# olegiy/manuscript-ocr

Hardware: NVIDIA B200
Metric: pages/sec (EAST decode+NMS+crop) (higher is better)
Workload: dtype f64 (NMS) / f32 (boxes) / u8 (crops)

## Files before the change

### manuscript-ocr_b200/csrc/crop.cu

```cuda
#include "crop_common.cuh"

namespace {

constexpr int kThreads = 224;
constexpr int kCtasPerSm = 4;
constexpr int kSlots = 3;
constexpr int kSrcBuf = 40 * 1024;
constexpr int kBandsY = 64, kCellsX = 8;

__device__ __forceinline__ void make_plan(const int32_t *cr, int n_pages, int img_h, int img_w, int ih, int iw,
                                          const uint8_t *pages, const uint8_t *const *page_ptrs,
                                          const int32_t *page_hw, Plan &p)
{
    plan_reset(p);
    p.page = cr[0];
    p.x1 = cr[1];
    p.y1 = cr[2];
    p.w = cr[3] - cr[1];
    p.h = cr[4] - cr[2];
    p.ok = p.page >= 0 && p.page < n_pages;
    if (!p.ok) return;
    const int H = page_ptrs ? page_hw[2 * p.page] : img_h, W = page_ptrs ? page_hw[2 * p.page + 1] : img_w;
    const uint8_t *page0 = page_ptrs ? page_ptrs[p.page] : pages + (size_t)p.page * img_h * (size_t)img_w * 3;
    p.ok = page0 != nullptr && H > 0 && W > 0 && p.w > 0 && p.h > 0 && p.x1 >= 0 && p.y1 >= 0 && cr[3] <= W && cr[4] <= H;
    if (!p.ok) return;
    const int w = p.w, h = p.h;
    plan_resize(w, h, ih, iw, p);
    const size_t stride = (size_t)W * 3;
    p.stride = (int)stride;
    p.src = page0 + (size_t)p.y1 * stride + (size_t)p.x1 * 3;
    const uintptr_t first = reinterpret_cast<uintptr_t>(p.src);
    const uintptr_t last_end = first + (size_t)(h - 1) * stride + (size_t)w * 3;
    const uintptr_t lo = reinterpret_cast<uintptr_t>(page_ptrs ? page0 : pages);
    const uintptr_t hi = page_ptrs ? lo + (size_t)H * stride : lo + (size_t)n_pages * img_h * (size_t)img_w * 3;
    const int mis = (stride & 15) == 0 ? (int)(first & 15) : 15;
    const int pitch = (mis + w * 3 + 15) & ~15;
    const bool fits = (size_t)pitch * h + 16 <= (size_t)kSrcBuf;
    const bool tail_ok = ((last_end + 15) & ~(uintptr_t)15) <= hi;
    if (fits && tail_ok && (lo & 15) == 0) {
        p.staged = 1;
        p.pitch = pitch;
    }
    p.fast = p.staged && p.w < 65536 && p.h < 65536 &&
             ((p.interp == 3 && p.scale_x < 2.999 && p.scale_y < 2.999) || (p.interp == 2 && p.isx == 2 && p.isy == 2));
}

__device__ __forceinline__ int crop_bucket(const Plan &p, const int32_t *page_hw, int img_h, int img_w, int n_pages)
{
    const int H = page_hw ? page_hw[2 * p.page] : img_h, W = page_hw ? page_hw[2 * p.page + 1] : img_w;
    const int by = min(kBandsY - 1, (int)(((int64_t)p.y1 * kBandsY) / max(H, 1)));
    const int bx = min(kCellsX - 1, (int)(((int64_t)p.x1 * kCellsX) / max(W, 1)));
    return (min(p.page, n_pages - 1) * kBandsY + by) * kCellsX + bx;
}

__global__ void __launch_bounds__(256) crop_plan_kernel(const uint8_t *__restrict__ pages,
                                                        const uint8_t *const *__restrict__ page_ptrs,
                                                        const int32_t *__restrict__ page_hw, int n_pages, int img_h,
                                                        int img_w, const int32_t *__restrict__ crops,
                                                        const int32_t *__restrict__ n_crops_dev,
                                                        const int32_t *__restrict__ range, int64_t crops_cap, int ih,
                                                        int iw, Plan *__restrict__ plans, int32_t *__restrict__ hist)
{
    ms_pdl_wait();
    int64_t begin = range ? range[0] : 0;
    int64_t n_crops = range ? range[1] : *n_crops_dev;
    if (n_crops > crops_cap) n_crops = crops_cap;
    for (int64_t i = begin + (int64_t)blockIdx.x * blockDim.x + threadIdx.x; i < n_crops;
         i += (int64_t)gridDim.x * blockDim.x) {
        Plan p;
        make_plan(crops + i * 5, n_pages, img_h, img_w, ih, iw, pages, page_ptrs, page_hw, p);
        plans[i] = p;
        if (p.fast) atomicAdd(&hist[crop_bucket(p, page_ptrs ? page_hw : nullptr, img_h, img_w, n_pages)], 1);
    }
}

__global__ void __launch_bounds__(1024) crop_bucket_scan_kernel(int32_t *__restrict__ hist, int n_buckets,
                                                                int32_t *__restrict__ n_work)
{
    ms_pdl_wait();
    __shared__ int s_warp[32];
    __shared__ int s_carry;
    const int lane = threadIdx.x & 31, warp = threadIdx.x >> 5;
    if (threadIdx.x == 0) s_carry = 0;
    __syncthreads();
    for (int tile = 0; tile < n_buckets; tile += 32 * 1024) {
        const int lo = tile + (int)threadIdx.x * 32;
        int v[32];
        if (lo + 32 <= n_buckets) {
            const int4 *q = reinterpret_cast<const int4 *>(hist + lo);
#pragma unroll
            for (int i = 0; i < 8; i++) {
                const int4 x = q[i];
                v[4 * i] = x.x, v[4 * i + 1] = x.y, v[4 * i + 2] = x.z, v[4 * i + 3] = x.w;
            }
        } else {
#pragma unroll
            for (int i = 0; i < 32; i++) v[i] = lo + i < n_buckets ? hist[lo + i] : 0;
        }
        int sum = 0;
#pragma unroll
        for (int i = 0; i < 32; i++) {
            const int c = v[i];
            v[i] = sum;
            sum += c;
        }
        int incl = sum;
#pragma unroll
        for (int o = 1; o < 32; o <<= 1) {
            const int u = __shfl_up_sync(0xffffffffu, incl, o);
            if (lane >= o) incl += u;
        }
        if (lane == 31) s_warp[warp] = incl;
        __syncthreads();
        const int carry = s_carry;
        if (warp == 0) {
            const int w = s_warp[lane];
            int wi = w;
#pragma unroll
            for (int o = 1; o < 32; o <<= 1) {
                const int u = __shfl_up_sync(0xffffffffu, wi, o);
                if (lane >= o) wi += u;
            }
            s_warp[lane] = wi - w;
            if (lane == 31) s_carry = carry + wi;
        }
        __syncthreads();
        const int base = carry + s_warp[warp] + incl - sum;
        if (lo + 32 <= n_buckets) {
            int4 *q = reinterpret_cast<int4 *>(hist + lo);
#pragma unroll
            for (int i = 0; i < 8; i++) q[i] = make_int4(base + v[4 * i], base + v[4 * i + 1], base + v[4 * i + 2], base + v[4 * i + 3]);
        } else {
#pragma unroll
            for (int i = 0; i < 32; i++)
                if (lo + i < n_buckets) hist[lo + i] = base + v[i];
        }
        __syncthreads();
    }
    if (threadIdx.x == 0) *n_work = s_carry;
}

__global__ void __launch_bounds__(256) crop_bucket_scatter_kernel(const Plan *__restrict__ plans,
                                                                  const int32_t *__restrict__ page_hw, int n_pages,
                                                                  int img_h, int img_w,
                                                                  const int32_t *__restrict__ n_crops_dev,
                                                                  const int32_t *__restrict__ range, int64_t crops_cap,
                                                                  int32_t *__restrict__ cursors, StageDesc *__restrict__ work)
{
    ms_pdl_wait();
    int64_t begin = range ? range[0] : 0;
    int64_t n_crops = range ? range[1] : *n_crops_dev;
    if (n_crops > crops_cap) n_crops = crops_cap;
    for (int64_t i = begin + (int64_t)blockIdx.x * blockDim.x + threadIdx.x; i < n_crops;
         i += (int64_t)gridDim.x * blockDim.x) {
        const Plan p = plans[i];
        if (p.fast) {
            StageDesc d;
            d.src = p.src;
            d.stride = p.stride;
            d.pitch = p.pitch;
            d.row_bytes = 3 * p.w;
            d.rows = p.h;
            d.ci = (int)i;
            work[atomicAdd(&cursors[crop_bucket(p, page_hw, img_h, img_w, n_pages)], 1)] = d;
        }
    }
}

constexpr int kProducerWarps = 2;
constexpr int kConsumerWarps = kThreads / 32 - kProducerWarps;

template <class T, bool kWriteU8>
__global__ void __launch_bounds__(kThreads, kCtasPerSm)
    crop_resize_pad_kernel(const Plan *__restrict__ plans, const StageDesc *__restrict__ work,
                           const int32_t *__restrict__ n_work_dev, int32_t *__restrict__ ticket, int ring_bytes, int ih,
                           int iw, T *__restrict__ batch, uint8_t *__restrict__ canvas_out, int vec_ok,
                           uint8_t *__restrict__ redo)
{
    ms_pdl_wait();
    extern __shared__ __align__(128) unsigned char smem[];
    const int tab_n = area_tab_words(ih, iw);
    uint32_t *tabs = reinterpret_cast<uint32_t *>(smem + ring_bytes);
    __shared__ StageSlots<kSlots> s_stage;
    __shared__ int s_meta[kSlots][8];

    const int warp = threadIdx.x >> 5, lane = threadIdx.x & 31;
    const int plane = ih * iw;
    stage_init(s_stage, kConsumerWarps);

    if (warp == 0) {
        stage_copy_warp(s_stage, smem, ring_bytes, work, *n_work_dev, ticket);
        return;
    }
    if (warp == 1) {
        for (int k = 0;; k++) {
            const int s = k % kSlots;
            const int ci = stage_wait_tick(s_stage, k);
            if (ci < 0) break;
            const Plan p = plans[ci];
            const bool two = p.interp == 2;
            const bool x3 = two || __all_sync(0xffffffffu, build_tables(p, tabs + (size_t)s * tab_n, tab_n, iw, lane));
            if (lane == 0) {
                s_meta[s][0] = p.nw;
                s_meta[s][1] = p.nh;
                s_meta[s][2] = p.y0;
                s_meta[s][3] = p.pitch;
                s_meta[s][4] = (int)(reinterpret_cast<uintptr_t>(p.src) & 15);
                s_meta[s][5] = p.stride & 15;
                s_meta[s][6] = two ? 2 : (x3 ? 1 : 0);
                s_meta[s][7] = strip_height<kConsumerWarps * 32>(p.nw, p.nh);
            }
            __syncwarp();
            if (lane == 0) mbar_arrive(&s_stage.full[s]);
            write_padding<T, kWriteU8>(p.nw, p.nh, p.y0, ih, iw, kHasBatch<T> ? batch + (size_t)ci * 3 * plane : nullptr,
                                               kWriteU8 ? canvas_out + (size_t)ci * 3 * plane : nullptr, vec_ok, lane, 32);
        }
        return;
    }

    const int ct = (warp - kProducerWarps) * 32 + lane;
    constexpr int kCT = kConsumerWarps * 32;
    for (int k = 0;; k++) {
        const int s = k % kSlots;
        const int64_t ci = stage_wait_full(s_stage, k);
        if (ci < 0) break;
        const int nw = s_meta[s][0], nh = s_meta[s][1], y0 = s_meta[s][2];
        const uint32_t pitch = (uint32_t)s_meta[s][3], a0 = (uint32_t)s_meta[s][4], sstep = (uint32_t)s_meta[s][5];
        const int G = s_meta[s][7];
        const uint32_t stage_off = (uint32_t)s_stage.off[s];
        T *dstf = kHasBatch<T> ? batch + (size_t)ci * 3 * plane : nullptr;
        uint8_t *dstu = kWriteU8 ? canvas_out + (size_t)ci * 3 * plane : nullptr;
        const uint32_t *tab = tabs + (size_t)s * tab_n;
        bool bad = false;
        if (s_meta[s][6] == 2)
            area2x2_pixels<T, kWriteU8, kCT>(smem, stage_off, pitch, a0, sstep, ih, iw, nw, nh, y0, dstf, dstu, ct);
        else if (sstep == 0)
            bad = s_meta[s][6] == 1 ? area4_strips<T, kWriteU8, kCT, 3, true>(smem, stage_off, pitch, a0, 0u, tab, tab_n, ih,
                                                                                 iw, nw, nh, y0, dstf, dstu, ct, G)
                               : area4_strips<T, kWriteU8, kCT, 4, true>(smem, stage_off, pitch, a0, 0u, tab, tab_n, ih,
                                                                                 iw, nw, nh, y0, dstf, dstu, ct, G);
        else
            bad = s_meta[s][6] == 1 ? area4_strips<T, kWriteU8, kCT, 3>(smem, stage_off, pitch, a0, sstep, tab, tab_n, ih, iw,
                                                                           nw, nh, y0, dstf, dstu, ct, G)
                               : area4_strips<T, kWriteU8, kCT, 4>(smem, stage_off, pitch, a0, sstep, tab, tab_n, ih, iw,
                                                                           nw, nh, y0, dstf, dstu, ct, G);
        if (bad) redo[ci] = 1;
        stage_release(s_stage, s);
    }
}

__global__ void __launch_bounds__(256) crop_generic_list_kernel(const Plan *__restrict__ plans,
                                                                const int32_t *__restrict__ n_crops_dev,
                                                                const int32_t *__restrict__ range, int64_t crops_cap,
                                                                const uint8_t *__restrict__ redo,
                                                                int32_t *__restrict__ list, int32_t *__restrict__ list_n)
{
    ms_pdl_wait();
    const int64_t begin = range ? range[0] : 0;
    int64_t n_crops = range ? range[1] : *n_crops_dev;
    if (n_crops > crops_cap) n_crops = crops_cap;
    for (int64_t ci = begin + (int64_t)blockIdx.x * blockDim.x + threadIdx.x; ci < n_crops;
         ci += (int64_t)gridDim.x * blockDim.x)
        if (!plans[ci].fast || redo[ci]) list[atomicAdd(list_n, 1)] = (int32_t)ci;
}

constexpr int kGenericMaxTab = 1024;

template <class T, bool kWriteU8>
__global__ void __launch_bounds__(256) crop_generic_kernel(const Plan *__restrict__ plans,
                                                           const int32_t *__restrict__ list,
                                                           const int32_t *__restrict__ list_n, int ih, int iw,
                                                           T *__restrict__ batch,
                                                           uint8_t *__restrict__ canvas_out, int vec_ok)
{
    ms_pdl_wait();
    __shared__ AxisEnt s_tab[kGenericMaxTab];
    const int plane = ih * iw;
    const int todo = *list_n;
    for (int li = blockIdx.x; li < todo; li += gridDim.x) {
        const int64_t ci = list[li];
        Plan p = plans[ci];
        if (!p.ok) p.nw = p.nh = 0;
        T *dstf = kHasBatch<T> ? batch + (size_t)ci * 3 * plane : nullptr;
        uint8_t *dstu = kWriteU8 ? canvas_out + (size_t)ci * 3 * plane : nullptr;
        write_padding<T, kWriteU8>(p, ih, iw, dstf, dstu, vec_ok, threadIdx.x, blockDim.x);
        const bool need_tab = p.ok && (p.interp == 1 || p.interp == 3);
        const bool tab_ok = need_tab && p.nw + p.nh <= kGenericMaxTab;
        __syncthreads();
        if (tab_ok) fill_axis_table(p, s_tab);
        __syncthreads();
        resample_canvas<T, kWriteU8>(p, PitchedSrc{p.src, (size_t)p.stride}, s_tab, tab_ok, need_tab, ih, iw, dstf,
                                             dstu);
    }
}

__global__ void __launch_bounds__(256) detector_input_kernel(const uint8_t *__restrict__ page, int H, int W, int th,
                                                             int tw, float *__restrict__ out_f32,
                                                             uint8_t *__restrict__ out_u8)
{
    ms_pdl_wait();
    const double scale_x = 1.0 / ((double)tw / (double)W), scale_y = 1.0 / ((double)th / (double)H);
    const bool same = (th == H && tw == W);
    const size_t plane = (size_t)th * tw;
    const PitchedSrc src{page, (size_t)W * 3};
    Plan p;
    p.interp = same ? 0 : 1;
    p.isx = p.isy = 0;
    for (size_t i = (size_t)blockIdx.x * blockDim.x + threadIdx.x; i < plane; i += (size_t)gridDim.x * blockDim.x) {
        const int dy = (int)(i / tw), dx = (int)(i - (size_t)dy * tw);
        AxisEnt ex = {}, ey = {};
        if (!same) {
            ex = linear_entry_x(dx, scale_x, W);
            ey = linear_entry_y(dy, scale_y, H);
        }
        unsigned char o0, o1, o2;
        resample_px(p, dx, dy, src, ex, ey, o0, o1, o2);
        if (out_f32) {
            out_f32[i] = ((float)o0 / 255.0f - 0.5f) / 0.5f;
            out_f32[plane + i] = ((float)o1 / 255.0f - 0.5f) / 0.5f;
            out_f32[2 * plane + i] = ((float)o2 / 255.0f - 0.5f) / 0.5f;
        }
        if (out_u8) {
            out_u8[i * 3] = o0;
            out_u8[i * 3 + 1] = o1;
            out_u8[i * 3 + 2] = o2;
        }
    }
}

}

int msk_detector_input(ms_ctx *ctx, const uint8_t *page, int img_h, int img_w, int target_h, int target_w,
                       float *out_f32, uint8_t *out_u8, cudaStream_t st)
{
    if (!page || img_h <= 0 || img_w <= 0 || target_h <= 0 || target_w <= 0 || (!out_f32 && !out_u8)) {
        ms_set_error("detector_input: bad arguments");
        return MS_ERR_INVALID;
    }
    const size_t n = (size_t)target_h * target_w;
    size_t grid = (n + 255) / 256;
    if (grid > (size_t)ctx->num_sms * 16) grid = (size_t)ctx->num_sms * 16;
    ms_launch(detector_input_kernel, (int)grid, 256, 0, st, page, img_h, img_w, target_h, target_w, out_f32, out_u8);
    MS_LAUNCH_CHECK(ctx);
    return MS_OK;
}

static size_t crop_bucket_count(int n_pages)
{
    size_t b = (size_t)(n_pages > 0 ? n_pages : 1) * kBandsY * kCellsX;
    return b > ((size_t)1 << 22) ? ((size_t)1 << 22) : b;
}

size_t msk_crop_scratch(int64_t crops_cap, int n_pages)
{
    const size_t n = (size_t)(crops_cap > 0 ? crops_cap : 0);
    return n * sizeof(Plan) + n + n * sizeof(int32_t) + n * sizeof(StageDesc) + crop_bucket_count(n_pages) * sizeof(int32_t) + 8192;
}

int msk_crop(ms_ctx *ctx, const uint8_t *pages, int n_pages, int img_h, int img_w, const int32_t *crops,
             const int32_t *n_crops, const int32_t *range, int64_t crops_cap, int out_h, int out_w, void *batch,
             int batch_dtype, uint8_t *canvas_u8, ms_bump bump, cudaStream_t st, const uint8_t *const *page_ptrs, const int32_t *page_hw)
{
    if (crops_cap <= 0 || n_pages <= 0) return MS_OK;
    const bool ragged = page_ptrs != nullptr && page_hw != nullptr;
    if (out_h <= 0 || out_w <= 0 || (!ragged && (img_h <= 0 || img_w <= 0 || !pages)) || (!batch && !canvas_u8)) {
        ms_set_error("crop: bad arguments");
        return MS_ERR_INVALID;
    }
    if ((int64_t)out_h * out_w > (1 << 20)) {
        ms_set_error("crop: canvas %dx%d too large", out_h, out_w);
        return MS_ERR_INVALID;
    }
    const size_t tab_bytes = (size_t)kSlots * (size_t)area_tab_words(out_h, out_w) * sizeof(uint32_t);
    const size_t min_ring = (size_t)kSrcBuf + 128;
    int per_sm = kCtasPerSm;
    while (per_sm > 1 && (227 * 1024) / per_sm < (int)(tab_bytes + min_ring + 1024 + 512)) per_sm--;
    if ((227 * 1024) / per_sm < (int)(tab_bytes + min_ring + 1024 + 512)) {
        ms_set_error("crop: canvas %dx%d needs %zu bytes of shared memory", out_h, out_w, tab_bytes + min_ring);
        return MS_ERR_INVALID;
    }
    size_t ring = ((size_t)(227 * 1024) / per_sm - 1024 - 512 - tab_bytes) & ~(size_t)127;
    if (ring > 96 * 1024) ring = 96 * 1024;
    const size_t smem = ring + tab_bytes;
    const int n_buckets = (int)crop_bucket_count(n_pages);
    Plan *plans = bump.take<Plan>((size_t)crops_cap);
    uint8_t *redo = bump.take<uint8_t>((size_t)crops_cap);
    int32_t *glist = bump.take<int32_t>((size_t)crops_cap);
    StageDesc *work = bump.take<StageDesc>((size_t)crops_cap);
    int32_t *hist = bump.take<int32_t>((size_t)n_buckets);
    int32_t *cnt = bump.take<int32_t>(4);
    if (!plans || !redo || !cnt) {
        ms_set_error("crop: scratch too small");
        return MS_ERR_CAPACITY;
    }
    int32_t *glist_n = cnt, *n_work = cnt + 1, *ticket = cnt + 2;
    MS_CUDA(cudaMemsetAsync(redo, 0, (size_t)crops_cap, st));
    MS_CUDA(cudaMemsetAsync(hist, 0, (size_t)n_buckets * sizeof(int32_t), st));
    MS_CUDA(cudaMemsetAsync(cnt, 0, 4 * sizeof(int32_t), st));
    int64_t lgrid = (crops_cap + 255) / 256;
    if (lgrid > (int64_t)ctx->num_sms * 8) lgrid = (int64_t)ctx->num_sms * 8;
    ms_launch(crop_plan_kernel, (int)lgrid, 256, 0, st, pages, ragged ? page_ptrs : nullptr, page_hw, n_pages, img_h, img_w, crops,
                                                 n_crops, range, crops_cap, out_h, out_w, plans, hist);
    MS_LAUNCH_CHECK(ctx);
    ms_launch(crop_bucket_scan_kernel, 1, 1024, 0, st, hist, n_buckets, n_work);
    MS_LAUNCH_CHECK(ctx);
    ms_launch(crop_bucket_scatter_kernel, (int)lgrid, 256, 0, st, plans, ragged ? page_hw : nullptr, n_pages, img_h, img_w, n_crops,
                                                           range, crops_cap, hist, work);
    MS_LAUNCH_CHECK(ctx);
    int64_t grid = (int64_t)ctx->num_sms * per_sm;
    if (grid > crops_cap) grid = crops_cap;
    int64_t ggrid = (int64_t)ctx->num_sms * 8;
    if (ggrid > crops_cap) ggrid = crops_cap;
    return launch_for_outputs(batch, batch_dtype, canvas_u8, [&](auto bt, auto u8) {
        using T = typename decltype(bt)::type;
        constexpr bool kU8 = decltype(u8)::value;
        T *out = static_cast<T *>(batch);
        const int vec_ok = batch_vec_ok<T>(batch, out_w);
        MS_TRY(ms_allow_smem(ctx, batch_slot<T, kU8>(MS_SMEM_CROP_U8), crop_resize_pad_kernel<T, kU8>, (int)smem));
        ms_launch(crop_resize_pad_kernel<T, kU8>, (int)grid, kThreads, smem, st, plans, work, n_work, ticket, (int)ring,
                  out_h, out_w, out, canvas_u8, vec_ok, redo);
        MS_LAUNCH_CHECK(ctx);
        ms_launch(crop_generic_list_kernel, (int)lgrid, 256, 0, st, plans, n_crops, range, crops_cap, redo, glist, glist_n);
        MS_LAUNCH_CHECK(ctx);
        ms_launch(crop_generic_kernel<T, kU8>, (int)ggrid, 256, 0, st, plans, glist, glist_n, out_h, out_w, out,
                  canvas_u8, vec_ok);
        MS_LAUNCH_CHECK(ctx);
        return MS_OK;
    });
}
```

### manuscript-ocr_b200/csrc/crop_common.cuh

```cuda
#pragma once
#include <cuda_bf16.h>
#include <cuda_fp16.h>

#include <type_traits>

#include "ms_internal.cuh"

namespace {

struct NoBatch {};
template <class T>
constexpr bool kHasBatch = !std::is_same<T, NoBatch>::value;

template <class T>
__device__ __forceinline__ T to_batch(float v);
template <>
__device__ __forceinline__ float to_batch<float>(float v) { return v; }
template <>
__device__ __forceinline__ __half to_batch<__half>(float v) { return __float2half_rn(v); }
template <>
__device__ __forceinline__ __nv_bfloat16 to_batch<__nv_bfloat16>(float v) { return __float2bfloat16_rn(v); }
__device__ __forceinline__ uint32_t batch_bits(__half v) { return __half_as_ushort(v); }
__device__ __forceinline__ uint32_t batch_bits(__nv_bfloat16 v) { return __bfloat16_as_ushort(v); }

template <class T>
__device__ __forceinline__ void store_norm(T *p, float v)
{
    __stcs(p, to_batch<T>((v - 127.5f) * (1.0f / 127.5f)));
}

__device__ __forceinline__ uint32_t smem_u32(const void *p) { return (uint32_t)__cvta_generic_to_shared(p); }

__device__ __forceinline__ void mbar_init(uint64_t *bar, int count)
{
    asm volatile("mbarrier.init.shared::cta.b64 [%0], %1;" ::"r"(smem_u32(bar)), "r"(count));
}
__device__ __forceinline__ void mbar_expect_tx(uint64_t *bar, uint32_t bytes)
{
    asm volatile("mbarrier.arrive.expect_tx.shared::cta.b64 _, [%0], %1;" ::"r"(smem_u32(bar)), "r"(bytes) : "memory");
}
__device__ __forceinline__ void mbar_wait(uint64_t *bar, uint32_t parity)
{
    asm volatile(
        "{\n"
        ".reg .pred p;\n"
        "mbarrier.try_wait.parity.shared::cta.b64 p, [%0], %1;\n"
        "@p bra DONE_%=;\n"
        "WAIT_%=:\n"
        "nanosleep.u32 %2;\n"
        "mbarrier.try_wait.parity.shared::cta.b64 p, [%0], %1;\n"
        "@!p bra WAIT_%=;\n"
        "DONE_%=:\n"
        "}\n" ::"r"(smem_u32(bar)),
        "r"(parity), "r"(100u)
        : "memory");
}
__device__ __forceinline__ void tma_bulk_g2s(void *dst_smem, const void *src_gmem, uint32_t bytes, uint64_t *bar)
{
    asm volatile("cp.async.bulk.shared::cluster.global.mbarrier::complete_tx::bytes [%0], [%1], %2, [%3];" ::"r"(
                     smem_u32(dst_smem)),
                 "l"(src_gmem), "r"(bytes), "r"(smem_u32(bar))
                 : "memory");
}
__device__ __forceinline__ void mbar_arrive(uint64_t *bar)
{
    asm volatile("mbarrier.arrive.shared::cta.b64 _, [%0];" ::"r"(smem_u32(bar)) : "memory");
}


struct __align__(16) StageDesc {
    const uint8_t *src;
    int stride;
    int pitch;
    int row_bytes;
    int rows;
    int ci;
};
static_assert(sizeof(StageDesc) == 32, "the copy warp loads a descriptor as two uint4");

template <int kSlots>
struct StageSlots {
    uint64_t full[kSlots], empty[kSlots], tick[kSlots];
    int ci[kSlots];
    int off[kSlots];
    int pitch[kSlots];
};

template <int kSlots>
__device__ __forceinline__ uint32_t stage_parity(int k)
{
    return (uint32_t)((k / kSlots) & 1);
}

template <int kSlots>
__device__ __forceinline__ void stage_init(StageSlots<kSlots> &ss, int consumer_warps)
{
    if (threadIdx.x == 0) {
#pragma unroll
        for (int i = 0; i < kSlots; i++) {
            mbar_init(&ss.full[i], 2);
            mbar_init(&ss.empty[i], consumer_warps);
            mbar_init(&ss.tick[i], 1);
        }
        asm volatile("fence.mbarrier_init.release.cluster;" ::: "memory");
    }
    __syncthreads();
}

template <int kSlots>
__device__ __forceinline__ void stage_copy_warp(StageSlots<kSlots> &ss, unsigned char *ring, int ring_bytes,
                                                const StageDesc *__restrict__ work, int n_work, int32_t *ticket)
{
    const int lane = threadIdx.x & 31;
    int q_off[kSlots], q_len[kSlots];
#pragma unroll
    for (int i = 0; i < kSlots; i++) q_off[i] = q_len[i] = 0;
    int head = 0;
    int oldest = 0;
    auto release_oldest = [&]() {
        mbar_wait(&ss.empty[oldest % kSlots], stage_parity<kSlots>(oldest));
        q_len[oldest % kSlots] = 0;
        oldest++;
    };
    auto load_desc = [&](int t) {
        StageDesc d;
        if (t < n_work) {
            const uint4 *q = reinterpret_cast<const uint4 *>(work + t);
            const uint4 a = q[0], b = q[1];
            d.src = reinterpret_cast<const uint8_t *>(((uint64_t)a.y << 32) | a.x);
            d.stride = (int)a.z;
            d.pitch = (int)a.w;
            d.row_bytes = (int)b.x;
            d.rows = (int)b.y;
            d.ci = (int)b.z;
        } else {
            d.src = nullptr;
            d.stride = d.pitch = d.row_bytes = d.rows = 0;
            d.ci = -1;
        }
        return d;
    };
    int t1 = 0;
    if (lane == 0) t1 = atomicAdd(ticket, 1);
    StageDesc cur = load_desc(__shfl_sync(0xffffffffu, t1, 0));
    if (lane == 0) t1 = atomicAdd(ticket, 1);
    for (int k = 0;; k++) {
        const int s = k % kSlots;
        const StageDesc nxt = load_desc(__shfl_sync(0xffffffffu, t1, 0));
        if (lane == 0 && cur.ci >= 0) t1 = atomicAdd(ticket, 1);
        while (oldest + kSlots <= k) release_oldest();
        if (cur.ci < 0) {
            if (lane == 0) {
                ss.ci[s] = -1;
                mbar_arrive(&ss.tick[s]);
                mbar_arrive(&ss.full[s]);
            }
            return;
        }
        const int need = (cur.pitch * cur.rows + 16 + 127) & ~127;
        int off;
        for (;;) {
            auto free_at = [&](int c) {
                bool ok = c + need <= ring_bytes;
#pragma unroll
                for (int i = 0; i < kSlots; i++) ok = ok && (q_len[i] == 0 || c + need <= q_off[i] || q_off[i] + q_len[i] <= c);
                return ok;
            };
            if (free_at(head)) {
                off = head;
                break;
            }
            if (free_at(0)) {
                off = 0;
                break;
            }
            release_oldest();
        }
        q_off[s] = off;
        q_len[s] = need;
        head = off + need;
        if (lane == 0) {
            ss.ci[s] = cur.ci;
            ss.off[s] = off;
            ss.pitch[s] = cur.pitch;
            mbar_arrive(&ss.tick[s]);
        }
        uint32_t bytes = 0;
        {
            const size_t stride = (size_t)cur.stride;
            unsigned char *buf = ring + off;
            for (int r = lane; r < cur.rows; r += 32) {
                const uint8_t *g = cur.src + (size_t)r * stride;
                const uint32_t a = (uint32_t)(reinterpret_cast<uintptr_t>(g) & 15);
                const uint32_t sz = (a + (uint32_t)cur.row_bytes + 15) & ~15u;
                tma_bulk_g2s(buf + (size_t)r * cur.pitch, g - a, sz, &ss.full[s]);
                bytes += sz;
            }
#pragma unroll
            for (int o = 16; o > 0; o >>= 1) bytes += __shfl_xor_sync(0xffffffffu, bytes, o);
        }
        if (lane == 0) mbar_expect_tx(&ss.full[s], bytes);
        cur = nxt;
    }
}

template <int kSlots>
__device__ __forceinline__ int stage_wait_tick(StageSlots<kSlots> &ss, int k)
{
    const int s = k % kSlots;
    mbar_wait(&ss.tick[s], stage_parity<kSlots>(k));
    const int ci = ss.ci[s];
    if (ci < 0 && (threadIdx.x & 31) == 0) mbar_arrive(&ss.full[s]);
    return ci;
}

template <int kSlots>
__device__ __forceinline__ int stage_wait_full(StageSlots<kSlots> &ss, int k)
{
    mbar_wait(&ss.full[k % kSlots], stage_parity<kSlots>(k));
    return ss.ci[k % kSlots];
}

template <int kSlots>
__device__ __forceinline__ void stage_release(StageSlots<kSlots> &ss, int s)
{
    __syncwarp();
    if ((threadIdx.x & 31) == 0) mbar_arrive(&ss.empty[s]);
}

struct Plan {
    int page, x1, y1, w, h;
    int nw, nh, y0;
    int interp;
    int isx, isy;
    int ok;
    int staged;
    int fast;
    int pitch;
    int stride;
    const uint8_t *src;
    double scale_x, scale_y;
};

__device__ __forceinline__ void plan_reset(Plan &p)
{
    p.page = p.x1 = p.y1 = p.w = p.h = 0;
    p.nw = p.nh = p.y0 = p.interp = p.isx = p.isy = 0;
    p.ok = p.staged = p.fast = p.pitch = p.stride = 0;
    p.src = nullptr;
    p.scale_x = p.scale_y = 1.0;
}

struct AxisEnt {
    int s0;
    int n;
    int nfirst;
    int nmid;
    float af, am, al;
    int pad;
};

__device__ __forceinline__ int cv_round(float v) { return __float2int_rn(v); }
__device__ __forceinline__ unsigned char sat_u8(int v) { return (unsigned char)min(max(v, 0), 255); }

__device__ __forceinline__ void plan_resize(int w, int h, int ih, int iw, Plan &p)
{
    double s1 = (double)ih / (double)max(h, 1), s2 = (double)iw / (double)max(w, 1);
// ... 337 lines not shown
    asm("mul.rn.f32x2 %0, %1, %2;" : "=l"(r) : "l"(a), "l"(b));
    return r;
}
__device__ __forceinline__ unsigned long long bytes2_f32(uint32_t va, uint32_t sa, uint32_t vb, uint32_t sb)
{
    const unsigned long long magic = f2_pack(-8388608.0f, -8388608.0f);
    return f2_add(f2_pack_bits(__byte_perm(va, 0x4B000000u, sa), __byte_perm(vb, 0x4B000000u, sb)), magic);
}

template <int kTaps>
__device__ __forceinline__ void hrow_area4(const unsigned char *smem_base, uint32_t o, const float4 wx, float &b0,
                                           float &b1, float &b2)
{
    const uint32_t *smem32 = reinterpret_cast<const uint32_t *>(smem_base);
    const uint32_t wi = o >> 2, sh = (o & 3u) * 8u;
    const uint32_t q0 = smem32[wi], q1 = smem32[wi + 1], q2 = smem32[wi + 2];
    const uint32_t q3 = kTaps > 3 ? smem32[wi + 3] : 0u;
    const uint32_t u0 = __funnelshift_r(q0, q1, sh), u1 = __funnelshift_r(q1, q2, sh), u2 = __funnelshift_r(q2, q3, sh);
    float p00, p01, p02, p10, p11, p12, p20, p21, p22;
    f2_unpack(f2_mul(bytes2_f32(u0, 0x7650, u0, 0x7651), f2_pack(wx.x, wx.x)), p00, p01);
    f2_unpack(f2_mul(bytes2_f32(u0, 0x7652, u0, 0x7653), f2_pack(wx.x, wx.y)), p02, p10);
    f2_unpack(f2_mul(bytes2_f32(u1, 0x7650, u1, 0x7651), f2_pack(wx.y, wx.y)), p11, p12);
    f2_unpack(f2_mul(bytes2_f32(u1, 0x7652, u1, 0x7653), f2_pack(wx.z, wx.z)), p20, p21);
    if (kTaps > 3) {
        float p30, p31, p32;
        f2_unpack(f2_mul(bytes2_f32(u2, 0x7650, u2, 0x7651), f2_pack(wx.z, wx.w)), p22, p30);
        f2_unpack(f2_mul(bytes2_f32(u2, 0x7652, u2, 0x7653), f2_pack(wx.w, wx.w)), p31, p32);
        b0 = ((p00 + p10) + p20) + p30;
        b1 = ((p01 + p11) + p21) + p31;
        b2 = ((p02 + p12) + p22) + p32;
    } else {
        p22 = byte_f32(u2, 0x7650) * wx.z;
        b0 = (p00 + p10) + p20;
        b1 = (p01 + p11) + p21;
        b2 = (p02 + p12) + p22;
    }
}

__host__ __device__ inline int area_tab_ybase(int iw) { return (5 * iw + 3) & ~3; }
__host__ __device__ inline int area_tab_words(int ih, int iw) { return area_tab_ybase(iw) + 8 * ih; }

__device__ __forceinline__ bool build_tables(const Plan &p, uint32_t *tab, int tab_n, int iw, int tid,
                                             int nthreads = 32)
{
    float *tw = reinterpret_cast<float *>(tab);
    bool x3 = true;
    const double inv_x = 1.0 / p.scale_x, inv_y = 1.0 / p.scale_y;
    for (int t = tid; t < p.nw + p.nh; t += nthreads) {
        const bool isx = t < p.nw;
        const int d = isx ? t : t - p.nw;
        const AxisEnt e = isx ? area_entry(d, p.scale_x, p.w, inv_x) : area_entry(d, p.scale_y, p.h, inv_y);
        const bool fits = e.n <= 4 && e.s0 >= 0 && e.s0 < 65536;
        x3 = x3 && !(isx && e.n > 3);
        const uint32_t packed = fits ? ((uint32_t)e.s0 | ((uint32_t)e.n << 16)) : 0xffff0000u;
        if (isx) {
            tab[d] = packed;
#pragma unroll
            for (int k = 0; k < 4; k++) tw[(size_t)(1 + k) * iw + d] = k < e.n ? area_weight(e, k) : 0.f;
        } else {
            uint32_t *rec = tab + area_tab_ybase(iw) + 8 * d;
            rec[0] = packed;
#pragma unroll
            for (int k = 0; k < 4; k++) reinterpret_cast<float *>(rec)[4 + k] = k < e.n ? area_weight(e, k) : 0.f;
        }
    }
    return x3;
}

template <int kCT>
__device__ __forceinline__ int strip_height(int nw, int nh)
{
    int G = 1, best = 0x7fffffff;
    for (int g = 8; g >= 1; g >>= 1) {
        const int items = ((nh + g - 1) / g) * nw;
        const int cost = ((items + kCT - 1) / kCT) * (2 * g + 1);
        if (cost < best) {
            best = cost;
            G = g;
        }
    }
    return G;
}

template <class T, bool kWriteU8, int kCT>
__device__ __forceinline__ void area2x2_pixels(const unsigned char *smem, uint32_t stage_off, uint32_t pitch, uint32_t a0,
                                               uint32_t sstep, int ih, int iw, int nw, int nh, int y0, T *dstf,
                                               uint8_t *dstu, int ct)
{
    const int plane = ih * iw;
    const uint32_t magic = 0xFFFFFFFFu / (uint32_t)nw + 1u;
    for (int t = ct; t < nw * nh; t += kCT) {
        const int dy = nw == 1 ? t : (int)__umulhi((uint32_t)t, magic), dx = t - dy * nw;
        int s0 = 0, s1 = 0, s2 = 0;
#pragma unroll
        for (int yy = 0; yy < 2; yy++) {
            const uint32_t r = (uint32_t)(2 * dy + yy);
            const unsigned char *row = smem + stage_off + r * pitch + ((a0 + r * sstep) & 15u) + 6u * (uint32_t)dx;
            s0 += row[0] + row[3];
            s1 += row[1] + row[4];
            s2 += row[2] + row[5];
        }
        const int o0 = (s0 + 2) >> 2, o1 = (s1 + 2) >> 2, o2 = (s2 + 2) >> 2;
        const int at = (y0 + dy) * iw + dx;
        if constexpr (kHasBatch<T>) {
            store_norm(dstf + at, (float)o0);
            store_norm(dstf + plane + at, (float)o1);
            store_norm(dstf + 2 * plane + at, (float)o2);
        }
        if (kWriteU8) {
            dstu[(size_t)at * 3] = (unsigned char)o0;
            dstu[(size_t)at * 3 + 1] = (unsigned char)o1;
            dstu[(size_t)at * 3 + 2] = (unsigned char)o2;
        }
    }
}

template <class T, bool kWriteU8, int kCT, int kTaps, bool kAligned = false>
__device__ __forceinline__ bool area4_strips(const unsigned char *smem, uint32_t stage_off, uint32_t pitch, uint32_t a0,
                                             uint32_t sstep, const uint32_t *tab, int tab_n, int ih, int iw, int nw,
                                             int nh, int y0, T *dstf, uint8_t *dstu, int ct, int G_in = 0,
                                             int dy_lo = 0, int dy_hi = -1)
{
    const int plane = ih * iw;
    const int G = G_in > 0 ? G_in : strip_height<kCT>(nw, nh);
    if (dy_hi < 0) dy_hi = nh;
    const int nitems = ((dy_hi - dy_lo + G - 1) / G) * nw;
    const uint32_t magic = 0xFFFFFFFFu / (uint32_t)nw + 1u;
    const float *tw = reinterpret_cast<const float *>(tab);
    bool bad = false;
    for (int t = ct; t < nitems; t += kCT) {
        const int grp = nw == 1 ? t : (int)__umulhi((uint32_t)t, magic), dx = t - grp * nw;
        const uint32_t px = tab[dx];
        bad = bad || (px >> 16) > 4u;
        const float4 wx = make_float4(tw[iw + dx], tw[2 * iw + dx], tw[3 * iw + dx], tw[4 * iw + dx]);
        const uint32_t xoff = stage_off + (px & 0xffffu) * 3u;
        int last_r = -1;
        float b0 = 0.f, b1 = 0.f, b2 = 0.f;
        const int dy_first = dy_lo + grp * G, dy_end = min(dy_hi, dy_first + G);
        T *orow = kHasBatch<T> ? dstf + (size_t)(y0 + dy_first) * iw + dx : nullptr;
        for (int dy = dy_first; dy < dy_end; dy++) {
            const uint32_t *yrec = tab + area_tab_ybase(iw) + 8 * dy;
            const uint32_t py = yrec[0];
            bad = bad || (py >> 16) > 4u;
            const int ys0 = (int)(py & 0xffffu), yn = min((int)(py >> 16), 4);
            const float4 wy4 = *reinterpret_cast<const float4 *>(yrec + 4);
            const float wyv[4] = {wy4.x, wy4.y, wy4.z, wy4.w};
            const uint32_t rbase = xoff + (uint32_t)ys0 * pitch;
            if (ys0 != last_r) {
                const uint32_t mis = (kAligned || sstep == 0) ? a0 : ((a0 + (uint32_t)ys0 * sstep) & 15u);
                hrow_area4<kTaps>(smem, rbase + mis, wx, b0, b1, b2);
            }
            float sum0 = wyv[0] * b0, sum1 = wyv[0] * b1, sum2 = wyv[0] * b2;
#pragma unroll
            for (int j = 1; j < 4; j++) {
                if (j < yn) {
                    const uint32_t r = (uint32_t)(ys0 + j);
                    const uint32_t mis = (kAligned || sstep == 0) ? a0 : ((a0 + r * sstep) & 15u);
                    hrow_area4<kTaps>(smem, rbase + (uint32_t)j * pitch + mis, wx, b0, b1, b2);
                    sum0 += wyv[j] * b0;
                    sum1 += wyv[j] * b1;
                    sum2 += wyv[j] * b2;
                }
            }
            last_r = ys0 + yn - 1;
            const float f0 = rintf(sum0), f1 = rintf(sum1), f2 = rintf(sum2);
            const int at = (y0 + dy) * iw + dx;
            if constexpr (kHasBatch<T>) {
                store_norm(orow, f0);
                store_norm(orow + plane, f1);
                store_norm(orow + 2 * plane, f2);
                orow += iw;
            }
            if (kWriteU8) {
                dstu[(size_t)at * 3] = sat_u8((int)f0);
                dstu[(size_t)at * 3 + 1] = sat_u8((int)f1);
                dstu[(size_t)at * 3 + 2] = sat_u8((int)f2);
            }
        }
    }
    return bad;
}

template <class T>
struct BatchType {
    using type = T;
};

template <class Launch>
int launch_for_outputs(const void *batch, int batch_dtype, const uint8_t *canvas_u8, Launch &&launch)
{
    if (!batch) return launch(BatchType<NoBatch>{}, std::true_type{});
    switch (batch_dtype) {
    case MS_DTYPE_F32:
        return canvas_u8 ? launch(BatchType<float>{}, std::true_type{}) : launch(BatchType<float>{}, std::false_type{});
    case MS_DTYPE_F16:
        return canvas_u8 ? launch(BatchType<__half>{}, std::true_type{}) : launch(BatchType<__half>{}, std::false_type{});
    case MS_DTYPE_BF16:
        return canvas_u8 ? launch(BatchType<__nv_bfloat16>{}, std::true_type{})
                         : launch(BatchType<__nv_bfloat16>{}, std::false_type{});
    }
    ms_set_error("crop: unknown batch dtype %d", batch_dtype);
    return MS_ERR_INVALID;
}

template <class T, bool kWriteU8>
constexpr ms_smem_slot batch_slot(ms_smem_slot first)
{
    const int t = std::is_same<T, float>::value ? 0 : std::is_same<T, __half>::value ? 1 : 2;
    return (ms_smem_slot)(first + (kHasBatch<T> ? 1 + 2 * t + (kWriteU8 ? 1 : 0) : 0));
}

template <class T>
int batch_vec_ok(const void *batch, int out_w)
{
    return (out_w % kBatchVec<T> == 0 && (reinterpret_cast<uintptr_t>(batch) & 15) == 0) ? 1 : 0;
}

}
```

Measured before the change: 28280.

## Stage resized crops in shared-memory tiles and add a dedicated canvas writer warp

Consumer warps now write resized pixels as bytes into a per-slot shared-memory tile instead of scattering normalized values straight to global memory. A new writer warp then streams the whole padded canvas (normalization, padding and u8 copy) with vectorized streaming stores, replacing the separate padding pass. The copy warp's ring allocator now reserves room for both the source and the tile, with extra barriers for tile completion and drain, and the block grows from 224 to 256 threads. This aims at coalesced global writes and at overlapping output writeback with compute. The cost is more shared memory per crop, so fewer crops take the fast staged path, plus added synchronization and a possible bottleneck on the single writer warp.

```diff
diff --git a/manuscript-ocr_b200/csrc/crop.cu b/manuscript-ocr_b200/csrc/crop.cu
--- a/manuscript-ocr_b200/csrc/crop.cu
+++ b/manuscript-ocr_b200/csrc/crop.cu
@@ -2,7 +2,7 @@
 
 namespace {
 
-constexpr int kThreads = 224;
+constexpr int kThreads = 256;
 constexpr int kCtasPerSm = 4;
 constexpr int kSlots = 3;
 constexpr int kSrcBuf = 40 * 1024;
@@ -10,7 +10,7 @@
 
 __device__ __forceinline__ void make_plan(const int32_t *cr, int n_pages, int img_h, int img_w, int ih, int iw,
                                           const uint8_t *pages, const uint8_t *const *page_ptrs,
-                                          const int32_t *page_hw, Plan &p)
+                                          const int32_t *page_hw, int ring_bytes, Plan &p)
 {
     plan_reset(p);
     p.page = cr[0];
@@ -35,7 +35,8 @@
     const uintptr_t hi = page_ptrs ? lo + (size_t)H * stride : lo + (size_t)n_pages * img_h * (size_t)img_w * 3;
     const int mis = (stride & 15) == 0 ? (int)(first & 15) : 15;
     const int pitch = (mis + w * 3 + 15) & ~15;
-    const bool fits = (size_t)pitch * h + 16 <= (size_t)kSrcBuf;
+    const bool fits = (size_t)pitch * h + 16 <= (size_t)ring_bytes &&
+                      stage_src_need(pitch, h) + stage_tile_need(tile_bytes(p.nw, p.nh)) <= ring_bytes;
     const bool tail_ok = ((last_end + 15) & ~(uintptr_t)15) <= hi;
     if (fits && tail_ok && (lo & 15) == 0) {
         p.staged = 1;
@@ -59,7 +60,8 @@
                                                         int img_w, const int32_t *__restrict__ crops,
                                                         const int32_t *__restrict__ n_crops_dev,
                                                         const int32_t *__restrict__ range, int64_t crops_cap, int ih,
-                                                        int iw, Plan *__restrict__ plans, int32_t *__restrict__ hist)
+                                                        int iw, int ring_bytes, Plan *__restrict__ plans,
+                                                        int32_t *__restrict__ hist)
 {
     ms_pdl_wait();
     int64_t begin = range ? range[0] : 0;
@@ -68,7 +70,7 @@
     for (int64_t i = begin + (int64_t)blockIdx.x * blockDim.x + threadIdx.x; i < n_crops;
          i += (int64_t)gridDim.x * blockDim.x) {
         Plan p;
-        make_plan(crops + i * 5, n_pages, img_h, img_w, ih, iw, pages, page_ptrs, page_hw, p);
+        make_plan(crops + i * 5, n_pages, img_h, img_w, ih, iw, pages, page_ptrs, page_hw, ring_bytes, p);
         plans[i] = p;
         if (p.fast) atomicAdd(&hist[crop_bucket(p, page_ptrs ? page_hw : nullptr, img_h, img_w, n_pages)], 1);
     }
@@ -162,12 +164,131 @@
             d.row_bytes = 3 * p.w;
             d.rows = p.h;
             d.ci = (int)i;
+            d.tile_bytes = tile_bytes(p.nw, p.nh);
             work[atomicAdd(&cursors[crop_bucket(p, page_hw, img_h, img_w, n_pages)], 1)] = d;
         }
     }
 }
 
-constexpr int kProducerWarps = 2;
+__device__ __forceinline__ void norm2(uint32_t va, uint32_t sa, uint32_t vb, uint32_t sb, float &lo, float &hi)
+{
+    const unsigned long long half = f2_pack(-127.5f, -127.5f), inv = f2_pack(1.0f / 127.5f, 1.0f / 127.5f);
+    f2_unpack(f2_mul(f2_add(bytes2_f32(va, sa, vb, sb), half), inv), lo, hi);
+}
+template <class T>
+__device__ __forceinline__ uint32_t pack2(float lo, float hi);
+template <>
+__device__ __forceinline__ uint32_t pack2<__half>(float lo, float hi)
+{
+    const __half2 h = __floats2half2_rn(lo, hi);
+    return *reinterpret_cast<const uint32_t *>(&h);
+}
+template <>
+__device__ __forceinline__ uint32_t pack2<__nv_bfloat16>(float lo, float hi)
+{
+    const __nv_bfloat162 h = __floats2bfloat162_rn(lo, hi);
+    return *reinterpret_cast<const uint32_t *>(&h);
+}
+template <int kW>
+__device__ __forceinline__ void pad_bytes(uint32_t (&w)[kW], int keep)
+{
+#pragma unroll
+    for (int j = 0; j < kW; j++) {
+        const int kb = keep - 4 * j;
+        if (kb < 4) w[j] |= kb <= 0 ? 0xFFFFFFFFu : 0xFFFFFFFFu << (8 * kb);
+    }
+}
+
+template <class T, bool kWriteU8>
+__device__ __forceinline__ void write_canvas(const unsigned char *tile, int nw, int nh, int y0, int ih, int iw, T *dstf,
+                                             uint8_t *dstu, int vec_ok, int lane)
+{
+    const uint32_t tp = (uint32_t)tile_pitch(nw);
+    if constexpr (kHasBatch<T>) {
+        if (vec_ok) {
+            constexpr int kV = kBatchVec<T>, kW = 3 * kV / 4;
+            const int V = iw / kV, n = ih * V;
+            uint4 *out = reinterpret_cast<uint4 *>(dstf);
+            int y = 0, v = lane;
+            while (v >= V) v -= V, y++;
+            for (int i = lane; i < n; i += 32) {
+                const int x = v * kV;
+                uint32_t w[kW];
+#pragma unroll
+                for (int j = 0; j < kW; j++) w[j] = 0xFFFFFFFFu;
+                if ((unsigned)(y - y0) < (unsigned)nh && x < nw) {
+                    const unsigned char *px = tile + (uint32_t)(y - y0) * tp + 3u * (uint32_t)x;
+                    if constexpr (kW == 6) {
+#pragma unroll
+                        for (int j = 0; j < 3; j++) {
+                            const uint2 q = reinterpret_cast<const uint2 *>(px)[j];
+                            w[2 * j] = q.x, w[2 * j + 1] = q.y;
+                        }
+                    } else {
+#pragma unroll
+                        for (int j = 0; j < kW; j++) w[j] = reinterpret_cast<const uint32_t *>(px)[j];
+                    }
+                    pad_bytes(w, 3 * (nw - x));
+                }
+#pragma unroll
+                for (int c = 0; c < 3; c++) {
+                    uint32_t o[4];
+#pragma unroll
+                    for (int e = 0; e < kV; e += 2) {
+                        constexpr int kSel = 0x7650;
+                        const int ka = 3 * e + c, kb = ka + 3;
+                        float lo, hi;
+                        norm2(w[ka >> 2], kSel | (ka & 3), w[kb >> 2], kSel | (kb & 3), lo, hi);
+                        if constexpr (sizeof(T) == 4) {
+                            o[e] = __float_as_uint(lo);
+                            o[e + 1] = __float_as_uint(hi);
+                        } else {
+                            o[e / 2] = pack2<T>(lo, hi);
+                        }
+                    }
+                    __stcs(out + (size_t)c * n + i, make_uint4(o[0], o[1], o[2], o[3]));
+                }
+                for (v += 32; v >= V; v -= V) y++;
+            }
+        } else {
+            for (int r = 0; r < 3 * ih; r++) {
+                const int c = r / ih, dy = r - c * ih - y0;
+                const bool in = (unsigned)dy < (unsigned)nh;
+                for (int x = lane; x < iw; x += 32) {
+                    const float b = in && x < nw ? (float)tile[(uint32_t)dy * tp + 3u * (uint32_t)x + (uint32_t)c] : 255.0f;
+                    __stcs(dstf + (size_t)r * iw + x, to_batch<T>((b - 127.5f) * (1.0f / 127.5f)));
+                }
+            }
+        }
+    }
+    if constexpr (kWriteU8) {
+        const int rb = 3 * iw;
+        if (rb % 16 == 0 && (reinterpret_cast<uintptr_t>(dstu) & 15) == 0) {
+            const int U = rb / 16, n = ih * U;
+            uint4 *out = reinterpret_cast<uint4 *>(dstu);
+            int y = 0, u = lane;
+            while (u >= U) u -= U, y++;
+            for (int i = lane; i < n; i += 32) {
+                const int b = u * 16;
+                uint32_t w[4] = {0xFFFFFFFFu, 0xFFFFFFFFu, 0xFFFFFFFFu, 0xFFFFFFFFu};
+                if ((unsigned)(y - y0) < (unsigned)nh && b < 3 * nw) {
+                    const uint4 q = *reinterpret_cast<const uint4 *>(tile + (uint32_t)(y - y0) * tp + (uint32_t)b);
+                    w[0] = q.x, w[1] = q.y, w[2] = q.z, w[3] = q.w;
+                    pad_bytes(w, 3 * nw - b);
+                }
+                out[i] = make_uint4(w[0], w[1], w[2], w[3]);
+                for (u += 32; u >= U; u -= U) y++;
+            }
+        } else {
+            for (int e = lane; e < ih * rb; e += 32) {
+                const int y = e / rb, b = e - y * rb, dy = y - y0;
+                dstu[e] = (unsigned)dy < (unsigned)nh && b < 3 * nw ? tile[(uint32_t)dy * tp + (uint32_t)b] : 255;
+            }
+        }
+    }
+}
+
+constexpr int kProducerWarps = 3;
 constexpr int kConsumerWarps = kThreads / 32 - kProducerWarps;
 
 template <class T, bool kWriteU8>
@@ -182,14 +303,16 @@
     const int tab_n = area_tab_words(ih, iw);
     uint32_t *tabs = reinterpret_cast<uint32_t *>(smem + ring_bytes);
     __shared__ StageSlots<kSlots> s_stage;
+    __shared__ StageTiles<kSlots> s_tiles;
     __shared__ int s_meta[kSlots][8];
 
     const int warp = threadIdx.x >> 5, lane = threadIdx.x & 31;
     const int plane = ih * iw;
+    stage_tiles_init(s_tiles, kConsumerWarps);
     stage_init(s_stage, kConsumerWarps);
 
     if (warp == 0) {
-        stage_copy_warp(s_stage, smem, ring_bytes, work, *n_work_dev, ticket);
+        stage_copy_warp<kSlots, true>(s_stage, smem, ring_bytes, work, *n_work_dev, ticket, &s_tiles);
         return;
     }
     if (warp == 1) {
@@ -199,7 +322,6 @@
             if (ci < 0) break;
             const Plan p = plans[ci];
             const bool two = p.interp == 2;
-            const bool x3 = two || __all_sync(0xffffffffu, build_tables(p, tabs + (size_t)s * tab_n, tab_n, iw, lane));
             if (lane == 0) {
                 s_meta[s][0] = p.nw;
                 s_meta[s][1] = p.nh;
@@ -207,13 +329,26 @@
                 s_meta[s][3] = p.pitch;
                 s_meta[s][4] = (int)(reinterpret_cast<uintptr_t>(p.src) & 15);
                 s_meta[s][5] = p.stride & 15;
-                s_meta[s][6] = two ? 2 : (x3 ? 1 : 0);
                 s_meta[s][7] = strip_height<kConsumerWarps * 32>(p.nw, p.nh);
             }
+            const bool x3 = two || __all_sync(0xffffffffu, build_tables(p, tabs + (size_t)s * tab_n, tab_n, iw, lane));
+            if (lane == 0) s_meta[s][6] = two ? 2 : (x3 ? 1 : 0);
             __syncwarp();
             if (lane == 0) mbar_arrive(&s_stage.full[s]);
-            write_padding<T, kWriteU8>(p.nw, p.nh, p.y0, ih, iw, kHasBatch<T> ? batch + (size_t)ci * 3 * plane : nullptr,
-                                               kWriteU8 ? canvas_out + (size_t)ci * 3 * plane : nullptr, vec_ok, lane, 32);
+        }
+        return;
+    }
+    if (warp == 2) {
+        for (int k = 0;; k++) {
+            const int s = k % kSlots;
+            mbar_wait(&s_tiles.done[s], stage_parity<kSlots>(k));
+            const int ci = s_stage.ci[s];
+            if (ci < 0) break;
+            write_canvas<T, kWriteU8>(smem + s_tiles.off[s], s_meta[s][0], s_meta[s][1], s_meta[s][2], ih, iw,
+                                      kHasBatch<T> ? batch + (size_t)ci * 3 * plane : nullptr,
+                                      kWriteU8 ? canvas_out + (size_t)ci * 3 * plane : nullptr, vec_ok, lane);
+            __syncwarp();
+            if (lane == 0) mbar_arrive(&s_tiles.drained[s]);
         }
         return;
     }
@@ -223,29 +358,35 @@
     for (int k = 0;; k++) {
         const int s = k % kSlots;
         const int64_t ci = stage_wait_full(s_stage, k);
-        if (ci < 0) break;
+        if (ci < 0) {
+            if (lane == 0) mbar_arrive(&s_tiles.done[s]);
+            break;
+        }
         const int nw = s_meta[s][0], nh = s_meta[s][1], y0 = s_meta[s][2];
         const uint32_t pitch = (uint32_t)s_meta[s][3], a0 = (uint32_t)s_meta[s][4], sstep = (uint32_t)s_meta[s][5];
         const int G = s_meta[s][7];
         const uint32_t stage_off = (uint32_t)s_stage.off[s];
-        T *dstf = kHasBatch<T> ? batch + (size_t)ci * 3 * plane : nullptr;
-        uint8_t *dstu = kWriteU8 ? canvas_out + (size_t)ci * 3 * plane : nullptr;
+        const ByteTile tile{smem + s_tiles.off[s], (uint32_t)tile_pitch(nw)};
         const uint32_t *tab = tabs + (size_t)s * tab_n;
         bool bad = false;
         if (s_meta[s][6] == 2)
-            area2x2_pixels<T, kWriteU8, kCT>(smem, stage_off, pitch, a0, sstep, ih, iw, nw, nh, y0, dstf, dstu, ct);
+            area2x2_pixels<T, kWriteU8, kCT>(smem, stage_off, pitch, a0, sstep, ih, iw, nw, nh, y0, nullptr, nullptr,
+                                             ct, tile);
         else if (sstep == 0)
-            bad = s_meta[s][6] == 1 ? area4_strips<T, kWriteU8, kCT, 3, true>(smem, stage_off, pitch, a0, 0u, tab, tab_n, ih,
-                                                                                 iw, nw, nh, y0, dstf, dstu, ct, G)
-                               : area4_strips<T, kWriteU8, kCT, 4, true>(smem, stage_off, pitch, a0, 0u, tab, tab_n, ih,
-                                                                                 iw, nw, nh, y0, dstf, dstu, ct, G);
+            bad = s_meta[s][6] == 1
+                      ? area4_strips<T, kWriteU8, kCT, 3, true>(smem, stage_off, pitch, a0, 0u, tab, tab_n, ih, iw, nw, nh,
+                                                                y0, nullptr, nullptr, ct, G, 0, -1, tile)
+                      : area4_strips<T, kWriteU8, kCT, 4, true>(smem, stage_off, pitch, a0, 0u, tab, tab_n, ih, iw, nw, nh,
+                                                                y0, nullptr, nullptr, ct, G, 0, -1, tile);
         else
-            bad = s_meta[s][6] == 1 ? area4_strips<T, kWriteU8, kCT, 3>(smem, stage_off, pitch, a0, sstep, tab, tab_n, ih, iw,
-                                                                           nw, nh, y0, dstf, dstu, ct, G)
-                               : area4_strips<T, kWriteU8, kCT, 4>(smem, stage_off, pitch, a0, sstep, tab, tab_n, ih, iw,
-                                                                           nw, nh, y0, dstf, dstu, ct, G);
+            bad = s_meta[s][6] == 1
+                      ? area4_strips<T, kWriteU8, kCT, 3>(smem, stage_off, pitch, a0, sstep, tab, tab_n, ih, iw, nw, nh,
+                                                          y0, nullptr, nullptr, ct, G, 0, -1, tile)
+                      : area4_strips<T, kWriteU8, kCT, 4>(smem, stage_off, pitch, a0, sstep, tab, tab_n, ih, iw, nw, nh,
+                                                          y0, nullptr, nullptr, ct, G, 0, -1, tile);
         if (bad) redo[ci] = 1;
         stage_release(s_stage, s);
+        if (lane == 0) mbar_arrive(&s_tiles.done[s]);
     }
 }
 
@@ -400,7 +541,7 @@
     int64_t lgrid = (crops_cap + 255) / 256;
     if (lgrid > (int64_t)ctx->num_sms * 8) lgrid = (int64_t)ctx->num_sms * 8;
     ms_launch(crop_plan_kernel, (int)lgrid, 256, 0, st, pages, ragged ? page_ptrs : nullptr, page_hw, n_pages, img_h, img_w, crops,
-                                                 n_crops, range, crops_cap, out_h, out_w, plans, hist);
+                                                 n_crops, range, crops_cap, out_h, out_w, (int)ring, plans, hist);
     MS_LAUNCH_CHECK(ctx);
     ms_launch(crop_bucket_scan_kernel, 1, 1024, 0, st, hist, n_buckets, n_work);
     MS_LAUNCH_CHECK(ctx);
diff --git a/manuscript-ocr_b200/csrc/crop_common.cuh b/manuscript-ocr_b200/csrc/crop_common.cuh
--- a/manuscript-ocr_b200/csrc/crop_common.cuh
+++ b/manuscript-ocr_b200/csrc/crop_common.cuh
@@ -75,8 +75,12 @@
     int row_bytes;
     int rows;
     int ci;
+    int tile_bytes;
 };
 static_assert(sizeof(StageDesc) == 32, "the copy warp loads a descriptor as two uint4");
+
+__host__ __device__ inline int stage_src_need(int pitch, int rows) { return (pitch * rows + 16 + 127) & ~127; }
+__host__ __device__ inline int stage_tile_need(int tile_bytes) { return (tile_bytes + 127) & ~127; }
 
 template <int kSlots>
 struct StageSlots {
@@ -87,6 +91,24 @@
 };
 
 template <int kSlots>
+struct StageTiles {
+    uint64_t done[kSlots], drained[kSlots];
+    int off[kSlots];
+};
+
+template <int kSlots>
+__device__ __forceinline__ void stage_tiles_init(StageTiles<kSlots> &st, int consumer_warps)
+{
+    if (threadIdx.x == 0) {
+#pragma unroll
+        for (int i = 0; i < kSlots; i++) {
+            mbar_init(&st.done[i], consumer_warps);
+            mbar_init(&st.drained[i], 1);
+        }
+    }
+}
+
+template <int kSlots>
 __device__ __forceinline__ uint32_t stage_parity(int k)
 {
     return (uint32_t)((k / kSlots) & 1);
@@ -107,20 +129,29 @@
     __syncthreads();
 }
 
-template <int kSlots>
+template <int kSlots, bool kTiles = false>
 __device__ __forceinline__ void stage_copy_warp(StageSlots<kSlots> &ss, unsigned char *ring, int ring_bytes,
-                                                const StageDesc *__restrict__ work, int n_work, int32_t *ticket)
+                                                const StageDesc *__restrict__ work, int n_work, int32_t *ticket,
+                                                StageTiles<kSlots> *tiles = nullptr)
 {
     const int lane = threadIdx.x & 31;
     int q_off[kSlots], q_len[kSlots];
-#pragma unroll
-    for (int i = 0; i < kSlots; i++) q_off[i] = q_len[i] = 0;
+    int t_off[kSlots], t_len[kSlots];
+#pragma unroll
+    for (int i = 0; i < kSlots; i++) q_off[i] = q_len[i] = t_off[i] = t_len[i] = 0;
     int head = 0;
     int oldest = 0;
+    int oldest_t = 0;
     auto release_oldest = [&]() {
         mbar_wait(&ss.empty[oldest % kSlots], stage_parity<kSlots>(oldest));
         q_len[oldest % kSlots] = 0;
         oldest++;
+    };
+    auto drain_oldest = [&]() {
+        mbar_wait(&tiles->drained[oldest_t % kSlots], stage_parity<kSlots>(oldest_t));
+        t_len[oldest_t % kSlots] = 0;
+        oldest_t++;
+        for (; oldest < oldest_t; oldest++) q_len[oldest % kSlots] = 0;
     };
     auto load_desc = [&](int t) {
         StageDesc d;
@@ -133,9 +164,10 @@
             d.row_bytes = (int)b.x;
             d.rows = (int)b.y;
             d.ci = (int)b.z;
+            d.tile_bytes = kTiles ? (int)b.w : 0;
         } else {
             d.src = nullptr;
-            d.stride = d.pitch = d.row_bytes = d.rows = 0;
+            d.stride = d.pitch = d.row_bytes = d.rows = d.tile_bytes = 0;
             d.ci = -1;
         }
         return d;
@@ -148,7 +180,11 @@
         const int s = k % kSlots;
         const StageDesc nxt = load_desc(__shfl_sync(0xffffffffu, t1, 0));
         if (lane == 0 && cur.ci >= 0) t1 = atomicAdd(ticket, 1);
-        while (oldest + kSlots <= k) release_oldest();
+        if constexpr (kTiles) {
+            while (oldest_t + kSlots <= k) drain_oldest();
+        } else {
+            while (oldest + kSlots <= k) release_oldest();
+        }
         if (cur.ci < 0) {
             if (lane == 0) {
                 ss.ci[s] = -1;
@@ -157,32 +193,62 @@
             }
             return;
         }
-        const int need = (cur.pitch * cur.rows + 16 + 127) & ~127;
-        int off;
+        const int need = stage_src_need(cur.pitch, cur.rows);
+        const int tneed = kTiles ? stage_tile_need(cur.tile_bytes) : 0;
+        int off, toff = 0;
         for (;;) {
-            auto free_at = [&](int c) {
-                bool ok = c + need <= ring_bytes;
-#pragma unroll
-                for (int i = 0; i < kSlots; i++) ok = ok && (q_len[i] == 0 || c + need <= q_off[i] || q_off[i] + q_len[i] <= c);
+            auto free_at = [&](int c, int n) {
+                bool ok = c + n <= ring_bytes;
+#pragma unroll
+                for (int i = 0; i < kSlots; i++) ok = ok && (q_len[i] == 0 || c + n <= q_off[i] || q_off[i] + q_len[i] <= c);
+                if constexpr (kTiles) {
+#pragma unroll
+                    for (int i = 0; i < kSlots; i++) ok = ok && (t_len[i] == 0 || c + n <= t_off[i] || t_off[i] + t_len[i] <= c);
+                }
                 return ok;
             };
-            if (free_at(head)) {
-                off = head;
-                break;
-            }
-            if (free_at(0)) {
-                off = 0;
-                break;
-            }
-            release_oldest();
+            if constexpr (kTiles) {
+                if (free_at(head, need + tneed)) {
+                    off = head, toff = head + need;
+                    break;
+                }
+                if (free_at(head, need) && tneed <= head && free_at(0, tneed)) {
+                    off = head, toff = 0;
+                    break;
+                }
+                if (free_at(0, need + tneed)) {
+                    off = 0, toff = need;
+                    break;
+                }
+                if (oldest < k)
+                    release_oldest();
+                else
+                    drain_oldest();
+            } else {
+                if (free_at(head, need)) {
+                    off = head;
+                    break;
+                }
+                if (free_at(0, need)) {
+                    off = 0;
+                    break;
+                }
+                release_oldest();
+            }
         }
         q_off[s] = off;
         q_len[s] = need;
         head = off + need;
+        if constexpr (kTiles) {
+            t_off[s] = toff;
+            t_len[s] = tneed;
+            head = max(head, toff + tneed);
+        }
         if (lane == 0) {
             ss.ci[s] = cur.ci;
             ss.off[s] = off;
             ss.pitch[s] = cur.pitch;
+            if constexpr (kTiles) tiles->off[s] = toff;
             mbar_arrive(&ss.tick[s]);
         }
         uint32_t bytes = 0;
@@ -686,10 +752,19 @@
     return G;
 }
 
-template <class T, bool kWriteU8, int kCT>
+struct NoTile {};
+struct ByteTile {
+    unsigned char *base;
+    uint32_t pitch;
+};
+__host__ __device__ inline int tile_pitch(int nw) { return (3 * nw + 15) & ~15; }
+__host__ __device__ inline int tile_bytes(int nw, int nh) { return nh * tile_pitch(nw) + 32; }
+__device__ __forceinline__ unsigned char f32_byte(float v) { return (unsigned char)__float_as_uint(v + 8388608.0f); }
+
+template <class T, bool kWriteU8, int kCT, class Tile = NoTile>
 __device__ __forceinline__ void area2x2_pixels(const unsigned char *smem, uint32_t stage_off, uint32_t pitch, uint32_t a0,
                                                uint32_t sstep, int ih, int iw, int nw, int nh, int y0, T *dstf,
-                                               uint8_t *dstu, int ct)
+                                               uint8_t *dstu, int ct, Tile tile = {})
 {
     const int plane = ih * iw;
     const uint32_t magic = 0xFFFFFFFFu / (uint32_t)nw + 1u;
@@ -706,25 +781,33 @@
         }
         const int o0 = (s0 + 2) >> 2, o1 = (s1 + 2) >> 2, o2 = (s2 + 2) >> 2;
         const int at = (y0 + dy) * iw + dx;
-        if constexpr (kHasBatch<T>) {
-            store_norm(dstf + at, (float)o0);
-            store_norm(dstf + plane + at, (float)o1);
-            store_norm(dstf + 2 * plane + at, (float)o2);
-        }
-        if (kWriteU8) {
-            dstu[(size_t)at * 3] = (unsigned char)o0;
-            dstu[(size_t)at * 3 + 1] = (unsigned char)o1;
-            dstu[(size_t)at * 3 + 2] = (unsigned char)o2;
-        }
-    }
-}
-
-template <class T, bool kWriteU8, int kCT, int kTaps, bool kAligned = false>
+        if constexpr (std::is_same<Tile, ByteTile>::value) {
+            unsigned char *px = tile.base + (uint32_t)dy * tile.pitch + 3u * (uint32_t)dx;
+            px[0] = (unsigned char)o0;
+            px[1] = (unsigned char)o1;
+            px[2] = (unsigned char)o2;
+        } else {
+            if constexpr (kHasBatch<T>) {
+                store_norm(dstf + at, (float)o0);
+                store_norm(dstf + plane + at, (float)o1);
+                store_norm(dstf + 2 * plane + at, (float)o2);
+            }
+            if (kWriteU8) {
+                dstu[(size_t)at * 3] = (unsigned char)o0;
+                dstu[(size_t)at * 3 + 1] = (unsigned char)o1;
+                dstu[(size_t)at * 3 + 2] = (unsigned char)o2;
+            }
+        }
+    }
+}
+
+template <class T, bool kWriteU8, int kCT, int kTaps, bool kAligned = false, class Tile = NoTile>
 __device__ __forceinline__ bool area4_strips(const unsigned char *smem, uint32_t stage_off, uint32_t pitch, uint32_t a0,
                                              uint32_t sstep, const uint32_t *tab, int tab_n, int ih, int iw, int nw,
                                              int nh, int y0, T *dstf, uint8_t *dstu, int ct, int G_in = 0,
-                                             int dy_lo = 0, int dy_hi = -1)
-{
+                                             int dy_lo = 0, int dy_hi = -1, Tile tile = {})
+{
+    constexpr bool kToTile = std::is_same<Tile, ByteTile>::value;
     const int plane = ih * iw;
     const int G = G_in > 0 ? G_in : strip_height<kCT>(nw, nh);
     if (dy_hi < 0) dy_hi = nh;
@@ -741,7 +824,9 @@
         int last_r = -1;
         float b0 = 0.f, b1 = 0.f, b2 = 0.f;
         const int dy_first = dy_lo + grp * G, dy_end = min(dy_hi, dy_first + G);
-        T *orow = kHasBatch<T> ? dstf + (size_t)(y0 + dy_first) * iw + dx : nullptr;
+        T *orow = kHasBatch<T> && !kToTile ? dstf + (size_t)(y0 + dy_first) * iw + dx : nullptr;
+        unsigned char *trow = nullptr;
+        if constexpr (kToTile) trow = tile.base + (uint32_t)dy_first * tile.pitch + 3u * (uint32_t)dx;
         for (int dy = dy_first; dy < dy_end; dy++) {
             const uint32_t *yrec = tab + area_tab_ybase(iw) + 8 * dy;
             const uint32_t py = yrec[0];
@@ -769,13 +854,18 @@
             last_r = ys0 + yn - 1;
             const float f0 = rintf(sum0), f1 = rintf(sum1), f2 = rintf(sum2);
             const int at = (y0 + dy) * iw + dx;
-            if constexpr (kHasBatch<T>) {
+            if constexpr (kToTile) {
+                trow[0] = f32_byte(f0);
+                trow[1] = f32_byte(f1);
+                trow[2] = f32_byte(f2);
+                trow += tile.pitch;
+            } else if constexpr (kHasBatch<T>) {
                 store_norm(orow, f0);
                 store_norm(orow + plane, f1);
                 store_norm(orow + 2 * plane, f2);
                 orow += iw;
             }
-            if (kWriteU8) {
+            if (kWriteU8 && !kToTile) {
                 dstu[(size_t)at * 3] = sat_u8((int)f0);
                 dstu[(size_t)at * 3 + 1] = sat_u8((int)f1);
                 dstu[(size_t)at * 3 + 2] = sat_u8((int)f2);
```

New measurement: 23010 (median of 6 runs). -18.6%, worse.
